# tg623623nana/Vehicle_Motion_Planning_with_Obstacles_Avoidance_using_MPC

Measured on AMD Instinct MI355X. Metric: OBCA MPC steps/sec (batch) at N=5, 3 obs, higher is better.
Workload: dtype f64

## Files before the change

### vehicle_motion_planning_with_obstacles_avoidance_using_mpc_amd/csrc/obca_device.h

```cpp
#ifndef OBCA_DEVICE_H
#define OBCA_DEVICE_H

#include <math.h>
#include <stdint.h>
#include "../../include/obca_mpc.h"

#define OBCA_ACC_MAX0 0.6
#define OBCA_ACC_MAX1 0.5235987755982988
#define OBCA_T_MIN 1e-4

#define OBCA_MU_INIT 0.1
#define OBCA_KAPPA_MU 0.2
#define OBCA_THETA_MU 1.5
#define OBCA_KAPPA_EPS 10.0
#define OBCA_TAU_MIN 0.99
#define OBCA_BOUND_PUSH 1e-2
#define OBCA_BOUND_FRAC 1e-2
#define OBCA_KAPPA_D 1e-5
#define OBCA_KAPPA_SIGMA 1e10
#define OBCA_S_MAX 100.0
#define OBCA_GAMMA_THETA 1e-5
#define OBCA_GAMMA_PHI 1e-8
#define OBCA_DELTA 1.0
#define OBCA_S_THETA 1.1
// ... 63 lines not shown
constexpr long long obca_even(long long c) { return (c + 1) & ~1ll; }
constexpr ObcaShapeSizes obca_shape_sizes(int N, int nO, int M) {
    const int N1 = N + 1, np = N1 * nO, MW = OBCA_MAX_EDGES + 6;
    const int n_max = N1 * (3 + M + 4 * nO) + 2 * N + 1;
    const int R_max = 3 + 3 * N + 3 + 2 * N1 + 2 * N + 2 * N + 2 + 2 * np + N1 * M + N1 * 4 * nO;
    long long t = 0;
    t += obca_even(n_max) + obca_even(n_max > 120 ? n_max : 120) + obca_even(5 * N1 + 1) + obca_even(n_max);
    t += 5 * obca_even(R_max);
    t += obca_even(3 * N1 + 3);
    t += 4 * obca_even(N1) + 2 * obca_even(2 * np);
    t += 3 * obca_even(2 * np);
    t += obca_even(N1 * M * 2) + obca_even(N1 * M) + obca_even(3 * N1);
    t += obca_even(36 * N1) + obca_even(8 * N1);
    {
        const long long nx = obca_even(n_max), nr = obca_even(R_max), ny = (long long)MW * 4 * np;
        t += obca_even(ny > nx + nr ? ny : nx + nr);
    }
    t += obca_even(36 * N1 > 12 * np ? 36 * N1 : 12 * np) + obca_even(6 * N1) + obca_even(12 * N1) + obca_even(2 * N1) + obca_even(9 * (N1 + 1));
    t += obca_even(32) + obca_even(8);
    const int inst_off = (int)t;
    t += OBCA_INST_DOUBLES;
    return ObcaShapeSizes{n_max, R_max, inst_off, t};
}
#define OBCA_LDS_CU_BYTES (160 * 1024)
#define OBCA_LDS_STATIC_BYTES 64
constexpr long long obca_soc_doubles(int N, int nO, int M) {
    return obca_even((long long)obca_shape_sizes(N, nO, M).n_max + 2 * (long long)obca_shape_sizes(N, nO, M).R_max + 2 * (long long)(N + 1) * nO);
}
constexpr int obca_wgs_per_cu(long long dyn_bytes, int cap) {
    return (int)(OBCA_LDS_CU_BYTES / (dyn_bytes + OBCA_LDS_STATIC_BYTES)) < cap ? (int)(OBCA_LDS_CU_BYTES / (dyn_bytes + OBCA_LDS_STATIC_BYTES)) : cap;
}
constexpr int obca_soc_lds_wave(int N, int nO, int M) {
    const long long base = 8 * obca_shape_sizes(N, nO, M).lds_doubles, with = base + 8 * obca_soc_doubles(N, nO, M);
    return (obca_wgs_per_cu(base, 4) > 0 && obca_wgs_per_cu(with, 4) == obca_wgs_per_cu(base, 4)) ? (int)obca_shape_sizes(N, nO, M).lds_doubles : 0;
}
constexpr int obca_soc_lds_mw(int N, int nO, int M) {
    const long long off = obca_shape_sizes(N, nO, M).lds_doubles + OBCA_ZK_DOUBLES(N) + OBCA_HYB_DOUBLES(obca_shape_sizes(N, nO, M).R_max);
    return 8 * (off + obca_soc_doubles(N, nO, M)) + OBCA_LDS_STATIC_BYTES <= OBCA_LDS_CU_BYTES ? (int)off : 0;
}
#define OBCA_SHAPES(X) X(5, 2, 2) X(5, 3, 6) X(5, 4, 10) X(5, 5, 14) X(5, 6, 18) X(6, 2, 2) X(6, 3, 6) X(6, 4, 10) X(6, 5, 14)
#define OBCA_MW_SHAPES(X) X(20, 3, 6) X(20, 5, 14)

struct ObcaWeightsDev { double Q[9], P[9], R1[4], R2[4]; };
struct ObcaOptsDev { double tol, rho, feas_tol; int32_t max_iter_free, max_iter_fixed, max_soc, order, nstarts, patience, retry_iter, dodge, screen, time_bound; };
static inline bool obca_resolve_starts(ObcaOptsDev* o, int start_order, int single_start, int patience, int retry_iter, int N, int dodge = 0, int terminal_screen = 0) {
    if (start_order < OBCA_START_DEFAULT || start_order > OBCA_START_X0_FIRST || single_start < 0 || single_start > 1) return false;
// ... 98 lines not shown
```

### vehicle_motion_planning_with_obstacles_avoidance_using_mpc_amd/csrc/obca_kernel.hip

```cpp

#include <hip/hip_runtime.h>
#include <stdint.h>
#include <math.h>
#include "obca_device.h"

#define SYNC() __syncthreads()

#ifndef OBCA_NT
#define OBCA_NT 64
#endif

#ifdef OBCA_PROFILE
#define PROF_DECL long long prof_last = wall_clock64();
#define PROF(i) { const long long t_ = wall_clock64(); prof_t[i] += t_ - prof_last; prof_last = t_; }
#define RPROF(i) { const long long t_ = wall_clock64(); prof_t[i] += t_ - rlast; rlast = t_; }
__device__ long long* prof_dummy;
#else
#define PROF_DECL
#define PROF(i)
#define RPROF(i)
#endif

namespace {

// ... 438 lines not shown
#undef X
    double* m_;
    double* gl_;
    enum {
#define X(f) K_##f,
        OBCA_ROW_FIELDS(X)
#undef X
        K_N };
    __device__ __forceinline__ static constexpr int slots() { return 5; }
#define X(f) __device__ __forceinline__ double& f##R(int j) { return j < 4 ? f##_[j] : m_[K_##f]; } \
             __device__ __forceinline__ double f##R(int j) const { return j < 4 ? f##_[j] : m_[K_##f]; }
    OBCA_ROW_FIELDS(X)
#undef X
#define X(f) __device__ __forceinline__ double& f(int j) { return f##R(j); } \
             __device__ __forceinline__ double f(int j) const { return f##R(j); }
    X(s) X(p) X(n) X(zL) X(zU) X(zp) X(zn) X(dy) X(iDs) X(iDp) X(iDn) X(rs) X(rp) X(rn)
#undef X
    __device__ __forceinline__ double& g(int j) { return j < 4 ? gl_[NT * j] : m_[K_g]; }
    __device__ __forceinline__ double g(int j) const { return j < 4 ? gl_[NT * j] : m_[K_g]; }
};

struct Err { double E, dual, prim, comp; };

template <int RPL>
__device__ __forceinline__ Err ipm_errors(const Lay& L, const Sh& S, const Rows<RPL>& W, double mu, double rho, double rxmax,
                          double crotmax, double nusum, int lane) {
    double dual = 0.0, prim = 0.0, comp = 0.0, ysum = 0.0, zsum = 0.0, nz = 0.0, nrow = 0.0;
#pragma unroll
    for (int j = 0; j < W.slots(); ++j) {
        const int r = lane + NT * j;
        if (r < L.R) {
            const double w = row_w(L, r);
            const bool eq = row_iseq(L, r);
            const double lo_ = S.Lb[r], up_ = S.Ub[r];
            const bool hasL = !eq && lo_ > -INFINITY, hasU = !eq && up_ < INFINITY;
            const double s = W.s(j), y = S.y[r], p = W.p(j), n = W.n(j);
            const double zL = hasL ? W.zL(j) : 0.0, zU = hasU ? W.zU(j) : 0.0, zp = W.zp(j), zn = W.zn(j);
            if (!eq) dual = dmaxabs(dual, -y - zL + zU);
            dual = dmaxabs(dual, rho - y - zp);
            dual = dmaxabs(dual, rho + y - zn);
            prim = dmaxabs(prim, W.g(j) - (eq ? 0.0 : s) - p + n);
            comp = dmaxabs(comp, p * zp - mu);
            comp = dmaxabs(comp, n * zn - mu);
            if (hasL) comp = dmaxabs(comp, (s - lo_) * zL - mu);
            if (hasU) comp = dmaxabs(comp, (up_ - s) * zU - mu);
            ysum += w * fabs(y);
            zsum += w * (zL + zU + zp + zn);
            nz += w * ((hasL ? 1.0 : 0.0) + (hasU ? 1.0 : 0.0) + 2.0);
            nrow += w;
        }
    }
    dual = fmax(red_max(dual), rxmax);
    prim = fmax(red_max(prim), crotmax);
    comp = red_max(comp);
    ysum = red_sum(ysum) + nusum;
    zsum = red_sum(zsum);
    nz = red_sum(nz);
    nrow = red_sum(nrow) + 2.0 * L.npair;
    const double sd = fmax(OBCA_S_MAX, (ysum + zsum) / (nrow + nz)) / OBCA_S_MAX;
    const double sc = fmax(OBCA_S_MAX, zsum / nz) / OBCA_S_MAX;
    Err e;
    e.dual = dual; e.prim = prim; e.comp = comp;
    e.E = fmax(fmax(dual / sd, prim), comp / sc);
    return e;
}

struct ErrFirst { Err e0, em; double th, pnsum, emax; };
template <int RPL>
__device__ __forceinline__ ErrFirst ipm_errors_first(const Lay& L, const Sh& S, const Rows<RPL>& W, double mu, double rho, double rxmax,
                                     double crotmax, double nusum, double th_lane, double nz, double nrow, int lane) {
    double dual = 0.0, prim = 0.0, comp0 = 0.0, compm = 0.0, ysum = 0.0, zsum = 0.0, th = th_lane, pnsum = 0.0, emax = 0.0;
#pragma unroll
    for (int j = 0; j < W.slots(); ++j) {
        const int r = lane + NT * j;
        if (r < L.R) {
            const double w = row_w(L, r);
            const bool eq = row_iseq(L, r);
            const double lo_ = S.Lb[r], up_ = S.Ub[r];
            const bool hasL = !eq && lo_ > -INFINITY, hasU = !eq && up_ < INFINITY;
            const double s = W.s(j), y = S.y[r], p = W.p(j), n = W.n(j);
            const double zL = hasL ? W.zL(j) : 0.0, zU = hasU ? W.zU(j) : 0.0, zp = W.zp(j), zn = W.zn(j);
            if (!eq) dual = dmaxabs(dual, -y - zL + zU);
            dual = dmaxabs(dual, rho - y - zp);
            dual = dmaxabs(dual, rho + y - zn);
            const double res = W.g(j) - (eq ? 0.0 : s) - p + n;
            prim = dmaxabs(prim, res);
            th += w * fabs(res);
            pnsum += w * (p + n);
            emax = fmax(emax, p + n);
            comp0 = dmaxabs(comp0, p * zp); compm = dmaxabs(compm, p * zp - mu);
            comp0 = dmaxabs(comp0, n * zn); compm = dmaxabs(compm, n * zn - mu);
            if (hasL) { comp0 = dmaxabs(comp0, (s - lo_) * zL); compm = dmaxabs(compm, (s - lo_) * zL - mu); }
            if (hasU) { comp0 = dmaxabs(comp0, (up_ - s) * zU); compm = dmaxabs(compm, (up_ - s) * zU - mu); }
            ysum += w * fabs(y);
            zsum += w * (zL + zU + zp + zn);
        }
    }
    ErrFirst o;
    dual = fmax(red_max(dual), rxmax);
    prim = fmax(red_max(prim), crotmax);
    comp0 = red_max(comp0);
    compm = red_max(compm);
    ysum = red_sum(ysum) + nusum;
    zsum = red_sum(zsum);
    o.th = red_sum(th); o.pnsum = red_sum(pnsum); o.emax = red_max(emax);
    const double sd = fmax(OBCA_S_MAX, (ysum + zsum) / (nrow + nz)) / OBCA_S_MAX;
    const double sc = fmax(OBCA_S_MAX, zsum / nz) / OBCA_S_MAX;
    o.e0.dual = dual; o.e0.prim = prim; o.e0.comp = comp0; o.e0.E = fmax(fmax(dual / sd, prim), comp0 / sc);
    o.em.dual = dual; o.em.prim = prim; o.em.comp = compm; o.em.E = fmax(fmax(dual / sd, prim), compm / sc);
    return o;
}

struct Lin { double iDs, iDp, iDn, rs, rp, rn; };
__device__ __forceinline__ Lin row_lin(double lo, double up, bool eq, double s, double p, double n, double y,
                                       double zL, double zU, double zp, double zn, double mu, double rho, double dw) {
    const bool hasL = !eq && lo > -INFINITY, hasU = !eq && up < INFINITY;
    double sig = 0.0, gs = 0.0;
    if (hasL) { const double isl = rcp64(s - lo); sig += zL * isl; gs -= mu * isl; }
    if (hasU) { const double isu = rcp64(up - s); sig += zU * isu; gs += mu * isu; }
    if (hasL && !hasU) gs += OBCA_KAPPA_D * mu;
    if (hasU && !hasL) gs -= OBCA_KAPPA_D * mu;
    const double ip = rcp64(p), inn = rcp64(n);
    Lin q;
    q.iDs = eq ? 0.0 : rcp64(sig + dw);
    q.iDp = rcp64(zp * ip + dw);
    q.iDn = rcp64(zn * inn + dw);
    q.rs = eq ? 0.0 : (-y + gs);
    q.rp = rho - y - mu * ip;
    q.rn = rho + y - mu * inn;
    return q;
}

__device__ __forceinline__ double row_barrier(double lo, double up, bool eq, double s, double p, double n, double mu,
// ... 968 lines not shown
template <bool FROM_MEMORY> __device__ __forceinline__ int uni(int v) { return FROM_MEMORY ? __builtin_amdgcn_readfirstlane(v) : v; }
template <bool FROM_MEMORY, class T> __device__ __forceinline__ T* uni(T* p) {
    if (!FROM_MEMORY) return p;
    const unsigned long long u = reinterpret_cast<unsigned long long>(p);
    const unsigned lo = (unsigned)__builtin_amdgcn_readfirstlane((int)(unsigned)u), hi = (unsigned)__builtin_amdgcn_readfirstlane((int)(unsigned)(u >> 32));
    return reinterpret_cast<T*>(((unsigned long long)hi << 32) | lo);
}
template <bool FROM_MEMORY> __device__ __forceinline__ double uni(double v) { return FROM_MEMORY ? lane_read(v, 0) : v; }
struct ObcaHead {
    int32_t B, N, nO, M, n_max, R_max, inst_off, two_sided, soc_lds;
    const int32_t* variant;
    const double *x0, *u0, *xref, *A, *b, *Ts, *term;
    double *xopt, *uopt, *ts_opt;
    int32_t *status, *iters;
    double *info, *prof, *warm_z;
    const int32_t* warm_use;
    double warm_mu;
    double *cert_z, *cert_y, *soc_ws, *gm_ws;
    long long gm_stride;
};

typedef const __attribute__((address_space(4))) ObcaLaunch ObcaLaunchConst;

struct ShapeAny { static constexpr bool fixed = false; static constexpr int N = 0, nO = 0, M = 0, n_max = 0, R_max = 0, inst_off = 0, soc_lds = 0; };
template <int N_, int NO_, int M_, bool FT = false>
struct ShapeIs {
    static constexpr bool fixed = true;
    static constexpr int N = N_, nO = NO_, M = M_;
    static constexpr int n_max = obca_shape_sizes(N_, NO_, M_).n_max, R_max = obca_shape_sizes(N_, NO_, M_).R_max - (FT ? 3 : 0),
                         inst_off = obca_shape_sizes(N_, NO_, M_).inst_off;
#if OBCA_NT == 64
    static constexpr int RPL = R_max <= 256 ? 4 : R_max <= 320 ? 5 : 6;
    static_assert(R_max <= 384, "shape beyond the one-wavefront kernels");
    static constexpr int soc_lds = obca_soc_lds_wave(N_, NO_, M_);
#else
    static constexpr int RPL = R_max <= 768 ? 3 : -5;
    static_assert(R_max <= 1280, "shape beyond the four-wavefront LDS kernels");
    static constexpr int soc_lds = obca_soc_lds_mw(N_, NO_, M_);
#endif
};

template <int RPL, bool FROM_MEMORY = false, class DESC = const ObcaLaunch, class SHAPE = ShapeAny>
__device__ __forceinline__ void obca_ipm_body(DESC& Ain, const int inst, const bool first) {
    extern __shared__ __attribute__((aligned(16))) double smem[];
    const int lane = threadIdx.x;
    ObcaHead A;
    {
        constexpr bool U = FROM_MEMORY;
        A.B = uni<U>(Ain.B); A.N = uni<U>(Ain.N); A.nO = uni<U>(Ain.nO); A.M = uni<U>(Ain.M); A.n_max = uni<U>(Ain.n_max);
        A.R_max = uni<U>(Ain.R_max); A.inst_off = uni<U>(Ain.inst_off); A.two_sided = uni<U>(Ain.two_sided); A.soc_lds = uni<U>(Ain.soc_lds);
        A.variant = uni<U>(Ain.variant); A.x0 = uni<U>(Ain.x0); A.u0 = uni<U>(Ain.u0); A.xref = uni<U>(Ain.xref); A.A = uni<U>(Ain.A);
// ... 40 lines not shown
    const bool dodge2 = start_s >= Ain.prm.opt.nstarts + 2;
    const bool from_window = kind == OBCA_KIND_WINDOW;

    Lay L;
    L.N = A.N; L.nO = A.nO; L.M = A.M;
    L.variant = A.variant[inst];
    L.free_T = (L.variant == 4) ? 1 : 0;
    L.NS = 5 + L.M + 4 * L.nO;
    L.n = (L.N + 1) * (3 + L.M + 4 * L.nO) + 2 * L.N + L.free_T;
    L.npair = (L.N + 1) * L.nO;
    L.r_init = 0; L.r_dyn = 3; L.r_term = 3 + 3 * L.N;
    L.r_xb = L.r_term + (L.variant == 4 ? 3 : 0);
    L.r_ub = L.r_xb + 2 * (L.N + 1);
    L.r_acc = L.r_ub + 2 * L.N;
    L.r_T = L.r_acc + 2 * L.N;
    L.r_tx = L.r_T + (L.free_T ? 2 : 0);
    L.r_norm = L.r_tx + (L.variant == 6 ? 2 : 0);
    L.r_dist = L.r_norm + L.npair;
    L.r_lam = L.r_dist + L.npair;
    L.r_mu = L.r_lam + (L.N + 1) * L.M;
    L.R = L.r_mu + (L.N + 1) * 4 * L.nO;

    constexpr bool GM = (RPL == 0);
    Sh S;
    Rows<RPL> W;
    {
        double* p = smem;
        double* q = nullptr;
        if constexpr (GM) q = A.gm_ws + (size_t)blockIdx.x * (size_t)A.gm_stride;
        auto take = [&](int cnt) { double* r = p; p += (cnt + 1) & ~1; return r; };
        auto takeG = [&](int cnt) { if constexpr (!GM) { double* r = p; p += (cnt + 1) & ~1; return r; } else { double* r = q; q += (cnt + 1) & ~1; return r; } };
        const int nmax = A.n_max, Rmax = A.R_max, np = L.npair, N1 = L.N + 1;
        S.x = takeG(nmax); S.dx = takeG(nmax > 120 ? nmax : 120); S.gf = take(5 * N1 + 1); S.bx = takeG(nmax);
        S.y = takeG(Rmax); S.Einv = takeG(Rmax); S.gh = takeG(Rmax); S.Lb = takeG(Rmax); S.Ub = takeG(Rmax); S.dy = take(3 * N1 + 3);
        S.ct = take(N1); S.st = take(N1); S.cc = takeG(2 * np); S.ctt = take(N1); S.stt = take(N1); S.cct = takeG(2 * np);
        S.nu = takeG(2 * np); S.dnu = takeG(2 * np); S.crot = takeG(2 * np);
        S.Aobs = takeG(N1 * L.M * 2); S.bobs = takeG(N1 * L.M); S.xref = take(3 * N1);
        S.Lall = take(36 * N1); S.lall = take(8 * N1);
        {
            const int nx = (nmax + 1) & ~1, nr = (Rmax + 1) & ~1, ny = MW * 4 * np;
            S.Y = takeG(ny > nx + nr ? ny : nx + nr);
            S.xt = S.Y; S.tmp = S.Y + nx;
        }
        if constexpr (!GM) {
            S.Pk = take(36 * N1 > 12 * np ? 36 * N1 : 12 * np);
            S.Sloc = S.Pk;
// ... 119 lines not shown
        gm = fmax(red_max(gm), O.rho);
        sf = (gm > OBCA_MAX_GRADIENT) ? OBCA_MAX_GRADIENT / gm : 1.0;
        rho = O.rho * sf;
    }
    SYNC();
    f0 = eval_objective<true>(L, S, in, S.x, sf, lane);
    PUT(IV_F, f0);
    double mu = (from_window || (kind >= OBCA_KIND_DODGE_R && !dodge2)) ? OBCA_RESTART_MU : (warm ? A.warm_mu : (dodge2 ? OBCA_DODGE_LEVEL2_MU : OBCA_MU_INIT));
    {
        int bb = 0;
        for (int r = lane; r < L.R; r += NT) {
            double lo, up;
            row_bounds(L, in, r, lo, up);
            S.Lb[r] = lo; S.Ub[r] = up;
            S.tmp[r] = row_value(L, S, in, S.x, S.ct, S.st, S.cc, r);
        }
#pragma unroll
        for (int j = 0; j < W.slots(); ++j) {
            const int r = lane + NT * j;
            W.s(j) = 0.0; W.p(j) = 1.0; W.n(j) = 1.0;
            W.zL(j) = 0.0; W.zU(j) = 0.0; W.zp(j) = 1.0; W.zn(j) = 1.0; W.g(j) = 0.0; W.dy(j) = 0.0;
            W.iDs(j) = 0.0; W.iDp(j) = 1.0; W.iDn(j) = 1.0; W.rs(j) = 0.0; W.rp(j) = 0.0; W.rn(j) = 0.0;
            if (r < L.R) {
                const double lo = S.Lb[r], up = S.Ub[r];
                const bool eq = row_iseq(L, r);
                const double g = S.tmp[r];
                double s = g;
                const bool hasL = lo > -INFINITY, hasU = up < INFINITY;
                if (eq) s = 0.0;
                else if (hasL && hasU) {
                    if (!(lo < up)) bb = 1;
                    const double pL = fmin(OBCA_BOUND_PUSH * fmax(1.0, fabs(lo)), OBCA_BOUND_FRAC * (up - lo));
                    const double pU = fmin(OBCA_BOUND_PUSH * fmax(1.0, fabs(up)), OBCA_BOUND_FRAC * (up - lo));
                    s = fmin(fmax(s, lo + pL), up - pU);
                } else if (hasL) s = fmax(s, lo + OBCA_BOUND_PUSH * fmax(1.0, fabs(lo)));
                else if (hasU) s = fmin(s, up - OBCA_BOUND_PUSH * fmax(1.0, fabs(up)));
                const double rr = g - s;
                const double a = (mu - rho * rr) / (2.0 * rho);
                const double en = a + sqrt(a * a + mu * rr / (2.0 * rho));
                const double ep = rr + en;
                W.g(j) = g; W.s(j) = s; W.p(j) = ep; W.n(j) = en;
                W.zp(j) = mu / ep; W.zn(j) = mu / en;
                W.zL(j) = (!eq && hasL) ? 1.0 : 0.0;
                W.zU(j) = (!eq && hasU) ? 1.0 : 0.0;
                S.y[r] = rho - mu / ep;
            }
        }
        bad_bounds = red_or(bb) != 0;
        for (int pr = lane; pr < L.npair; pr += NT) {
            double e1, e2;
            rot_value(L, S.x, S.ct, S.st, S.cc, pr, e1, e2);
            S.crot[2 * pr] = e1; S.crot[2 * pr + 1] = e2;
        }
        SYNC();
    }

    double cnt_nz = 0.0, cnt_rows = 0.0;
#pragma unroll
    for (int j = 0; j < W.slots(); ++j) {
        const int r = lane + NT * j;
        if (r < L.R) {
            const double w = row_w(L, r);
            const bool eq = row_iseq(L, r);
            cnt_nz += w * (((!eq && S.Lb[r] > -INFINITY) ? 1.0 : 0.0) + ((!eq && S.Ub[r] < INFINITY) ? 1.0 : 0.0) + 2.0);
            cnt_rows += w;
        }
    }
    cnt_nz = red_sum(cnt_nz);
    cnt_rows = red_sum(cnt_rows) + 2.0 * L.npair;
    PUT(IV_CNTNZ, cnt_nz); PUT(IV_CNTROWS, cnt_rows);

    bool f_valid = false;
    double f_th = 0.0, f_phi = 0.0;
    PUT(IV_TAU, fmax(OBCA_TAU_MIN, 1.0 - mu));
    PUT(IV_DWLAST, 0.0); PUT(IV_EMAX, 0.0); PUT(IV_PHIK, NAN);
    int acc_count = 0;
    bool have_prev = false;

#ifdef OBCA_PROFILE
    long long prof_t[20];
    for (int i = 0; i < 20; ++i) prof_t[i] = 0;
#endif
    enum { LS_TH = 0, LS_FOBJ, LS_DW, LS_AZ, LS_DPHI, LS_PHI, LS_AMIN, LS_PWTH, LS_PWDPHI, LS_ALPHA, LS_THOLD };
    bool soc_pass = false, use_soc = false, first_trial = true;
    int soc_it = 0;
    PROF_DECL
#ifdef OBCA_PROFILE
    if (NT == 64) prof_t[10] += prof_last - prof_body_t0;
#endif
    if (bad_bounds) status = OBCA_STATUS_BAD_BOUNDS;
    else
    for (it = 0; it <= max_iter; ++it) {
        PROF(11)
        double th = 0.0, fobj = 0.0, delta_w = 0.0;
        if (!soc_pass) {
        gather_grad<false>(L, S, in, S.bx, lane);
        double rxmax = 0.0, crotmax = 0.0, nusum = 0.0, pnsum = 0.0;
        for (int t = lane; t < L.n; t += NT) rxmax = dmaxabs(rxmax, S.bx[t]);
        for (int t = lane; t < 2 * L.npair; t += NT) { crotmax = dmaxabs(crotmax, S.crot[t]); nusum += fabs(S.nu[t]); th += fabs(S.crot[t]); }
        rxmax = red_max(rxmax); crotmax = red_max(crotmax); nusum = red_sum(nusum);
        const ErrFirst ef = ipm_errors_first<RPL>(L, S, W, mu, rho, rxmax, crotmax, nusum, th, GET(IV_CNTNZ), GET(IV_CNTROWS), lane);
        th = ef.th; pnsum = ef.pnsum; PUT(IV_EMAX, ef.emax);
        const Err e0 = ef.e0;
        const double E0 = e0.E;
        PUT(IV_E0, E0);
        if (it == 0) {
            PUT(IV_THMAX, OBCA_THETA_MAX_FACT * fmax(1.0, th));
            PUT(IV_THMIN, OBCA_THETA_MIN_FACT * fmax(1.0, th));
        }
        if (E0 <= O.tol && e0.dual <= 1.0 && e0.prim <= 1e-4 && e0.comp <= 1e-4) { status = OBCA_STATUS_OK; break; }
        fobj = GET(IV_F) + rho * pnsum;
        const double objchg = have_prev ? fabs(fobj - GET(IV_FPREV)) / fmax(1.0, fabs(fobj)) : INFINITY;
        if (E0 <= acc_tol && e0.dual <= 1e10 && e0.prim <= 1e-2 && e0.comp <= 1e-2 && objchg <= acc_objchg) {
            if (++acc_count >= OBCA_ACCEPTABLE_ITER) { status = OBCA_STATUS_ACCEPTABLE; break; }
        } else acc_count = 0;
        if (it == max_iter) break;
        PROF(0)
        {
            const double mu_floor = O.tol / (OBCA_KAPPA_EPS + 1.0);
            bool first_mu = true;
            while (mu > mu_floor) {
                const Err em = first_mu ? ef.em : ipm_errors<RPL>(L, S, W, mu, rho, rxmax, crotmax, nusum, lane);
                first_mu = false;
                if (em.E > OBCA_KAPPA_EPS * mu) break;
                mu = fmax(mu_floor, fmin(OBCA_KAPPA_MU * mu, mu * sqrt(mu)));
                PUT(IV_TAU, fmax(OBCA_TAU_MIN, 1.0 - mu));
                PUT(IV_PHIK, NAN);
                f_valid = false;
            }
        }
        } else {
            th = S.lsv[LS_TH]; fobj = S.lsv[LS_FOBJ]; delta_w = S.lsv[LS_DW];
            (void)eval_objective<true>(L, S, in, S.x, sf, lane);
        }
        PROF(1)
#define ws_dxo (A.soc_lds ? smem + A.soc_lds : A.soc_ws + (size_t)inst * (A.n_max + 2 * A.R_max + 2 * L.npair))
#define ws_dyo (ws_dxo + A.n_max)
#define ws_gsoc (ws_dyo + A.R_max)
#define ws_dnuo (ws_gsoc + A.R_max)
        const int max_soc = (A.soc_lds || A.soc_ws) ? O.max_soc : 0;
#pragma unroll
        for (int j = 0; j < W.slots(); ++j) {
            W.dy(j) = 0.0; W.iDs(j) = 0.0; W.iDp(j) = 0.0; W.iDn(j) = 0.0; W.rs(j) = 0.0; W.rp(j) = 0.0; W.rn(j) = 0.0;
        }
        bool first_try = true;
        int fail = 0;
        const double dw_last = GET(IV_DWLAST);
        for (;;) {
#pragma unroll
            for (int j = 0; j < W.slots(); ++j) {
                const int r = lane + NT * j;
                if (r < L.R) {
                    const bool eq = row_iseq(L, r);
                    const double y = S.y[r];
                    const double lo_ = S.Lb[r], up_ = S.Ub[r];
                    const Lin q = row_lin(lo_, up_, eq, W.s(j), W.p(j), W.n(j), y, W.zL(j), W.zU(j), W.zp(j),
                                          W.zn(j), mu, rho, delta_w);
                    const double rg = soc_pass ? ws_gsoc[r] : W.g(j) - (eq ? 0.0 : W.s(j)) - W.p(j) + W.n(j);
                    const double gh = rg + q.rs * q.iDs + q.rp * q.iDp - q.rn * q.iDn;
                    const double Ei = rcp64(q.iDs + q.iDp + q.iDn);
                    S.Einv[r] = Ei;
                    S.gh[r] = gh;
                    S.tmp[r] = row_soft(L, r) ? y : fma(gh, Ei, y);
                }
            }
            SYNC();
            if constexpr (GM) {
                double* es = const_cast<double*>(S.Es); double* gs = const_cast<double*>(S.gs); double* uv = const_cast<double*>(S.uv);
                for (int t = lane; t < L.r_term; t += NT) { es[t] = S.Einv[t]; gs[t] = S.gh[t]; }
                for (int t = lane; t < 2 * L.N; t += NT) uv[t] = S.x[L.iu(t >> 1) + (t & 1)];
                if (lane == 0 && L.free_T) uv[2 * (L.N + 1)] = S.x[L.iT()];
                SYNC();
            }
            gather_grad<true>(L, S, in, S.bx, lane);
            PROF(2)
            assemble_stages(L, S, in, sf, delta_w, lane);
            PROF(3)
            int bad = local_blocks(L, S, in, delta_w, lane);
            PROF(4)
#ifdef OBCA_PROFILE
            if (!bad) bad = riccati(L, S, in, lane, prof_t, A.two_sided != 0);
#if !defined(OBCA_TWO_SIDED_CHECK) && OBCA_NT >= 256
            if (A.two_sided != 0) {
                double dmax = 0.0;
                for (int r = L.r_init + (lane & 63); r < L.r_term; r += 64) dmax = fmax(dmax, S.Einv[r]);
                dmax = wave_max(dmax);
// ... 29 lines not shown
#endif
#else
            if (!bad) bad = riccati(L, S, in, lane, A.two_sided != 0);
#endif
            PROF(5)
            ++nfact;
            if (!bad || soc_pass) break;
            if (first_try) {
                delta_w = (dw_last == 0.0) ? OBCA_DELTA_W_0 : fmax(OBCA_DELTA_W_MIN, OBCA_KAPPA_W_MINUS * dw_last);
                first_try = false;
            } else {
                delta_w *= (dw_last == 0.0) ? OBCA_KAPPA_W_PLUS_BAR : OBCA_KAPPA_W_PLUS;
            }
            if (delta_w > OBCA_DELTA_W_MAX) { fail = 1; break; }
        }
        if (fail) { status = OBCA_STATUS_NUMERIC; break; }
        if (!soc_pass && delta_w > 0.0) PUT(IV_DWLAST, delta_w);
        double a_max = 1.0, a_z = 1.0, dphi = 0.0, phi = 0.0;
        const double phik = GET(IV_PHIK);
        const bool phi_known = !soc_pass && isfinite(phik);
        const double tau = GET(IV_TAU);
        for (int r = lane; r < L.R; r += NT)
            S.tmp[r] = row_soft(L, r) ? S.dy[r] : (row_jdx(L, S, in, r) + S.gh[r]) * S.Einv[r];
#pragma unroll
        for (int j = 0; j < W.slots(); ++j) {
            const int r = lane + NT * j;
            if (r < L.R) {
                const bool eq = row_iseq(L, r);
                const double lo_ = S.Lb[r], up_ = S.Ub[r];
            const bool hasL = !eq && lo_ > -INFINITY, hasU = !eq && up_ < INFINITY;
                const double dy = S.tmp[r];
                W.dy(j) = dy;
                {
                    const Lin q = row_lin(lo_, up_, eq, W.s(j), W.p(j), W.n(j), S.y[r], W.zL(j), W.zU(j), W.zp(j),
                                          W.zn(j), mu, rho, delta_w);
                    W.iDs(j) = q.iDs; W.iDp(j) = q.iDp; W.iDn(j) = q.iDn; W.rs(j) = q.rs; W.rp(j) = q.rp; W.rn(j) = q.rn;
                }
                const double w = row_w(L, r);
                const double ds = (dy - W.rs(j)) * W.iDs(j);
                const double dp = (dy - W.rp(j)) * W.iDp(j);
                const double dn = (-dy - W.rn(j)) * W.iDn(j);
                const double s = W.s(j), p = W.p(j), n = W.n(j);
                double gs = eq ? 0.0 : W.rs(j) + S.y[r];
                const double ids = rcp64(ds), ip = rcp64(p), inn = rcp64(n);
                if (hasL) {
                    const double sl = s - lo_, zL = W.zL(j);
                    if (ds < 0.0) a_max = fmin(a_max, -tau * sl * ids);
                    const double dz = (mu - zL * ds) * rcp64(sl) - zL;
                    if (dz < 0.0) a_z = fmin(a_z, -tau * zL * rcp64(dz));
                }
                if (hasU) {
                    const double su = up_ - s, zU = W.zU(j);
                    if (ds > 0.0) a_max = fmin(a_max, tau * su * ids);
                    const double dz = (mu + zU * ds) * rcp64(su) - zU;
                    if (dz < 0.0) a_z = fmin(a_z, -tau * zU * rcp64(dz));
                }
                if (dp < 0.0) a_max = fmin(a_max, -tau * p * rcp64(dp));
                if (dn < 0.0) a_max = fmin(a_max, -tau * n * rcp64(dn));
                const double zp = W.zp(j), zn = W.zn(j);
                const double dzp = (mu - zp * dp) * ip - zp, dzn = (mu - zn * dn) * inn - zn;
                if (dzp < 0.0) a_z = fmin(a_z, -tau * zp * rcp64(dzp));
                if (dzn < 0.0) a_z = fmin(a_z, -tau * zn * rcp64(dzn));
                if (!phi_known) phi += w * row_barrier(lo_, up_, eq, s, p, n, mu, rho);
                dphi += w * (gs * ds + (rho - mu * ip) * dp + (rho - mu * inn) * dn);
            }
        }
        for (int t = lane; t < L.n; t += NT) {
            const int k = t / L.NS, q = t - k * L.NS;
            if (L.free_T && t == L.iT()) dphi += S.gf[L.igT()] * S.dx[t];
            else if (q < (k < L.N ? 5 : 3)) dphi += S.gf[L.ig(k) + q] * S.dx[t];
        }
        a_max = red_min(a_max); a_z = red_min(a_z); dphi = red_sum(dphi); phi = phi_known ? phik : red_sum(phi) + GET(IV_F);
        double alpha_min;
        double pw_th = 0.0, pw_dphi = 1.0;
        double alpha = a_max, a_try = a_max, th_old = 0.0;
        if (!soc_pass) {
            if (dphi < 0.0) {
                pw_th = dpow(th, OBCA_S_THETA);
                pw_dphi = dpow(-dphi, OBCA_S_PHI);
                double c = fmin(OBCA_GAMMA_THETA, OBCA_GAMMA_PHI * th / (-dphi));
                if (th <= GET(IV_THMIN)) c = fmin(c, OBCA_DELTA * pw_th / pw_dphi);
                alpha_min = OBCA_GAMMA_ALPHA * c;
            } else alpha_min = OBCA_GAMMA_ALPHA * OBCA_GAMMA_THETA;
            first_trial = true; use_soc = false; soc_it = 0;
        } else {
            a_try = a_max;
            a_z = S.lsv[LS_AZ]; dphi = S.lsv[LS_DPHI]; phi = S.lsv[LS_PHI]; alpha_min = S.lsv[LS_AMIN];
            pw_th = S.lsv[LS_PWTH]; pw_dphi = S.lsv[LS_PWDPHI]; alpha = S.lsv[LS_ALPHA]; th_old = S.lsv[LS_THOLD];
        }
        soc_pass = false;
        PROF(6)
        double f_t = 0.0, phi_acc = NAN;
        bool accepted = false, aug = false;
        for (;;) {
            for (int t = lane; t < L.n; t += NT) S.xt[t] = S.x[t] + a_try * S.dx[t];
            SYNC();
            eval_geom(L, S, S.xt, S.ctt, S.stt, S.cct, lane);
            f_t = eval_objective<true>(L, S, in, S.xt, sf, lane);
            double th_t = 0.0, phi_t = 0.0;
            for (int r = lane; r < L.R; r += NT) S.tmp[r] = row_value(L, S, in, S.xt, S.ctt, S.stt, S.cct, r);
#pragma unroll
            for (int j = 0; j < W.slots(); ++j) {
                const int r = lane + NT * j;
                if (r < L.R) {
                    const bool eq = row_iseq(L, r);
                    const double dy = W.dy(j), w = row_w(L, r);
                    const double lo_ = S.Lb[r], up_ = S.Ub[r];
                    const double st = eq ? 0.0 : W.s(j) + a_try * (dy - W.rs(j)) * W.iDs(j);
                    const double pt = W.p(j) + a_try * (dy - W.rp(j)) * W.iDp(j);
                    const double nt = W.n(j) + a_try * (-dy - W.rn(j)) * W.iDn(j);
                    const double gt = S.tmp[r];
                    th_t += w * fabs(gt - st - pt + nt);
                    phi_t += w * row_barrier(lo_, up_, eq, st, pt, nt, mu, rho);
                }
            }
            for (int pr = lane; pr < L.npair; pr += NT) {
                double e1, e2;
                rot_value(L, S.xt, S.ctt, S.stt, S.cct, pr, e1, e2);
                th_t += fabs(e1) + fabs(e2);
                S.bx[2 * pr] = e1; S.bx[2 * pr + 1] = e2;
            }
            th_t = red_sum(th_t);
            phi_t = red_sum(phi_t) + f_t;
            bool ok = false;
            aug = false;
            const bool finite = isfinite(phi_t) && isfinite(th_t);
#if OBCA_NT == 64
            const bool blocked = (th_t >= GET(IV_THMAX)) || (__any(f_valid && th_t >= f_th && phi_t >= f_phi) != 0);
#else
            const bool blocked = (th_t >= GET(IV_THMAX)) || red_or(f_valid && th_t >= f_th && phi_t >= f_phi);
// ... 12 lines not shown
            bool soc_start = false, soc_next = false;
            if (use_soc) {
                if (!fin_eval || th_t > OBCA_KAPPA_SOC * th_old || soc_it >= max_soc) {
                    for (int t = lane; t < L.n; t += NT) S.dx[t] = ws_dxo[t];
                    for (int t = lane; t < 2 * L.npair; t += NT) S.dnu[t] = ws_dnuo[t];
#pragma unroll
                    for (int j = 0; j < W.slots(); ++j) {
                        const int r = lane + NT * j;
                        if (r < L.R) W.dy(j) = ws_dyo[r];
                    }
                    use_soc = false;
                    SYNC();
                } else soc_next = true;
            } else if (first_trial && max_soc > 0 && fin_eval && th_t >= th) {
                soc_start = true;
            }
            first_trial = false;
            if (soc_start || soc_next) {
                const double cf = soc_start ? alpha : a_try;
#pragma unroll
                for (int j = 0; j < W.slots(); ++j) {
                    const int r = lane + NT * j;
                    if (r < L.R) {
                        const bool eq = row_iseq(L, r);
                        const double dy = W.dy(j);
                        const double st = eq ? 0.0 : W.s(j) + a_try * (dy - W.rs(j)) * W.iDs(j);
                        const double pt = W.p(j) + a_try * (dy - W.rp(j)) * W.iDp(j);
                        const double nt = W.n(j) + a_try * (-dy - W.rn(j)) * W.iDn(j);
                        const double res = S.tmp[r] - st - pt + nt;
                        const double old = soc_start ? W.g(j) - (eq ? 0.0 : W.s(j)) - W.p(j) + W.n(j) : ws_gsoc[r];
                        ws_gsoc[r] = cf * old + res;
                        if (soc_start) ws_dyo[r] = dy;
                    }
                }
                if (soc_start) {
                    for (int t = lane; t < L.n; t += NT) ws_dxo[t] = S.dx[t];
                    for (int t = lane; t < 2 * L.npair; t += NT) ws_dnuo[t] = S.dnu[t];
                }
                for (int t = lane; t < 2 * L.npair; t += NT) S.crot[t] = cf * S.crot[t] + S.bx[t];
                if (lane == 0) {
                    S.lsv[LS_TH] = th; S.lsv[LS_FOBJ] = fobj; S.lsv[LS_DW] = delta_w; S.lsv[LS_AZ] = a_z; S.lsv[LS_DPHI] = dphi;
                    S.lsv[LS_PHI] = phi; S.lsv[LS_AMIN] = alpha_min; S.lsv[LS_PWTH] = pw_th; S.lsv[LS_PWDPHI] = pw_dphi;
                    S.lsv[LS_ALPHA] = alpha; S.lsv[LS_THOLD] = th_t;
                }
                use_soc = true;
                soc_pass = true;
                ++soc_it;
// ... 10 lines not shown
        if (!accepted) { status = OBCA_STATUS_LINESEARCH; break; }
        if (aug) {
            const double tn = (1.0 - OBCA_GAMMA_THETA) * th, pn = phi - OBCA_GAMMA_PHI * th;
#if OBCA_NT == 64
            if (f_valid && f_th >= tn && f_phi >= pn) f_valid = false;
            const unsigned long long freem = __ballot(!f_valid);
            if (freem == 0ull) { status = OBCA_STATUS_NUMERIC; break; }
            const int slot = __ffsll((long long)freem) - 1;
            if (lane == slot) { f_valid = true; f_th = tn; f_phi = pn; }
#else
            if (f_valid && f_th >= tn && f_phi >= pn) f_valid = false;
            const unsigned long long freem = __ballot(!f_valid && lane < OBCA_FILTER_CAP(A.R_max));
            const double cand = freem ? (double)((lane & ~63) + __ffsll((long long)freem) - 1) : 1e9;
            const double slot = red_min(cand);
            const int full = slot > 1e8 ? 1 : 0;
            if (!full && lane == (int)slot) { f_valid = true; f_th = tn; f_phi = pn; }
            if (full) { status = OBCA_STATUS_NUMERIC; break; }
#endif
        }
#pragma unroll
        for (int j = 0; j < W.slots(); ++j) {
            const int r = lane + NT * j;
            if (r < L.R) {
                const bool eq = row_iseq(L, r);
                const double lo_ = S.Lb[r], up_ = S.Ub[r];
            const bool hasL = !eq && lo_ > -INFINITY, hasU = !eq && up_ < INFINITY;
                const double dy = W.dy(j);
                const double dyz = use_soc ? ws_dyo[r] : dy;
                const double ds = (dy - W.rs(j)) * W.iDs(j);
                const double dp = (dy - W.rp(j)) * W.iDp(j);
                const double dn = (-dy - W.rn(j)) * W.iDn(j);
                const double dsz = (dyz - W.rs(j)) * W.iDs(j);
                const double dpz = (dyz - W.rp(j)) * W.iDp(j);
                const double dnz = (-dyz - W.rn(j)) * W.iDn(j);
                const double lo = lo_, up = up_;
                const double s_old = W.s(j), p_old = W.p(j), n_old = W.n(j);
                const double s = eq ? 0.0 : s_old + a_try * ds, p = p_old + a_try * dp, n = n_old + a_try * dn;
                const double ks = OBCA_KAPPA_SIGMA, iks = 1.0 / OBCA_KAPPA_SIGMA;
                if (hasL) {
                    const double zL = W.zL(j) + a_z * ((mu - W.zL(j) * dsz) * rcp64(s_old - lo) - W.zL(j));
                    const double msl = mu * rcp64(s - lo);
                    W.zL(j) = fmax(fmin(zL, ks * msl), msl * iks);
                }
                if (hasU) {
                    const double zU = W.zU(j) + a_z * ((mu + W.zU(j) * dsz) * rcp64(up - s_old) - W.zU(j));
                    const double msu = mu * rcp64(up - s);
                    W.zU(j) = fmax(fmin(zU, ks * msu), msu * iks);
                }
                const double zp = W.zp(j) + a_z * ((mu - W.zp(j) * dpz) * rcp64(p_old) - W.zp(j));
// ... 198 lines not shown
#ifndef OBCA_LOOP_R4
#define OBCA_LOOP_R4 true
#endif
#ifndef OBCA_LOOP_R56
#define OBCA_LOOP_R56 true
#endif
#ifndef OBCA_LOOP_MW
#define OBCA_LOOP_MW false
#endif
#ifndef OBCA_LOOP_GM
#define OBCA_LOOP_GM true
#endif
#if OBCA_NT == 64 && defined(OBCA_TU_SHAPE)
#ifndef OBCA_SHAPE_KERNEL_ATTR
#define OBCA_SHAPE_KERNEL_ATTR
#endif
#define OBCA_DEFINE_SHAPE_KERNEL(N_, O_, M_)                                                                                   \
    extern "C" __global__ void __launch_bounds__(64) OBCA_SHAPE_KERNEL_ATTR obca_ipm_kernel_s##N_##_##O_##_##M_(ObcaLaunch A, ObcaLaunch A2, ObcaLaunch A3) { \
        using SH = ShapeIs<N_, O_, M_>;                                                                                        \
        solve_with_escalation<SH::RPL, true, true, SH>(A, A2, A3);                                                            \
    }
OBCA_TU_SHAPE(OBCA_DEFINE_SHAPE_KERNEL)
#elif OBCA_NT == 64
extern "C" __global__ void __launch_bounds__(64) obca_ipm_kernel_r4(ObcaLaunch A, ObcaLaunch A2, ObcaLaunch A3) { solve_with_escalation<4, OBCA_LOOP_R4>(A, A2, A3); }
extern "C" __global__ void __launch_bounds__(64) obca_ipm_kernel_r5(ObcaLaunch A, ObcaLaunch A2, ObcaLaunch A3) { solve_with_escalation<5, OBCA_LOOP_R56>(A, A2, A3); }
extern "C" __global__ void __launch_bounds__(64) obca_ipm_kernel_r6(ObcaLaunch A, ObcaLaunch A2, ObcaLaunch A3) { solve_with_escalation<6, OBCA_LOOP_R56>(A, A2, A3); }
extern "C" __global__ void __launch_bounds__(64) obca_ipm_kernel_gm1(ObcaLaunch A, ObcaLaunch A2, ObcaLaunch A3) { solve_with_escalation<0, OBCA_LOOP_GM>(A, A2, A3); }

#include "obca_rollout_core.h"
#include "obca_audit_core.h"

__device__ __noinline__ void ro_prepare(const rollout::Dev* D, int b) { rollout::prepare(*D, b); }
__device__ __noinline__ void ro_finish(const rollout::Dev* D, int b) { rollout::finish(*D, b); }
__device__ __noinline__ void ro_stop(const rollout::Dev* D, int b) { rollout::stop_check_wave(*D, b); }
__device__ __noinline__ int ro_screen(const ObcaLaunch* L, int b, double* tmax) { return terminal_screen_dev(L, b, 0, 1, tmax); }
__device__ __noinline__ int ro_retry(const rollout::Dev* D, int g, int b) { rollout::make_retry(*D, g, b); return D->var8[g][b]; }
__device__ __noinline__ long long ro_flag_sel(const rollout::Dev* D, int b) { return ((long long)D->sel[b] << 32) | (unsigned)D->flags[b]; }


#define OBCA_RO_SPIN_LIMIT (1 << 24)
#define OBCA_GETREG_XCC_ID (20 | (0 << 6) | ((4 - 1) << 11))

template <int RPL, class SHAPE>
__device__ __forceinline__ void ro_solve_step(const rollout::Dev& D, const ObcaLaunch* launches, const int g, const int b, int* ro_msg) {
    const int lane = threadIdx.x;
    bool nodge = false;
// ... 165 lines not shown
```

Measured before the change: 1.128 million.

## Specialize mu-only row slots at compile time and reuse error terms in mu loop

For fixed shapes, the register slot index from which all rows are known to be the mu/obstacle rows (no equality, lower bound 0, no upper bound, weight 1, not soft) is computed at compile time. Row loops skip the LDS loads of bounds, weights and row flags for those slots. The mu-decrease loop now recomputes only the complementarity error and reuses the dual and primal terms from the first error evaluation, since those do not depend on mu. The power computations for the switching condition are done once on lane 0 and only when needed. The approach relies on the row-layout assumption holding for every shape variant.

```diff
diff --git a/vehicle_motion_planning_with_obstacles_avoidance_using_mpc_amd/csrc/obca_device.h b/vehicle_motion_planning_with_obstacles_avoidance_using_mpc_amd/csrc/obca_device.h
--- a/vehicle_motion_planning_with_obstacles_avoidance_using_mpc_amd/csrc/obca_device.h
+++ b/vehicle_motion_planning_with_obstacles_avoidance_using_mpc_amd/csrc/obca_device.h
@@ -109,6 +109,20 @@
     t += OBCA_INST_DOUBLES;
     return ObcaShapeSizes{n_max, R_max, inst_off, t};
 }
+#define OBCA_NO_MU_SLOT (1 << 20)
+constexpr int obca_r_mu(int N, int nO, int M, int variant) {
+    return 3 + 3 * N + (variant == 4 ? 3 : 0) + 2 * (N + 1) + 2 * N + 2 * N + (variant == 4 ? 2 : 0) + (variant == 6 ? 2 : 0) +
+           2 * (N + 1) * nO + (N + 1) * M;
+}
+constexpr int obca_mu_slot(int N, int nO, int M, int nt) {
+    int r = obca_r_mu(N, nO, M, 4);
+    if (obca_r_mu(N, nO, M, 6) > r) r = obca_r_mu(N, nO, M, 6);
+    if (obca_r_mu(N, nO, M, 8) > r) r = obca_r_mu(N, nO, M, 8);
+    return (r + nt - 1) / nt;
+}
+static_assert(obca_mu_slot(5, 3, 6, 64) == 2 && obca_mu_slot(6, 3, 6, 64) == 3 && obca_mu_slot(5, 2, 2, 64) == 2 &&
+              obca_mu_slot(5, 5, 14, 64) == 4 && obca_mu_slot(5, 6, 18, 64) == 4, "mu slots of the one-wavefront shapes");
+static_assert(obca_mu_slot(20, 3, 6, 256) == 2 && obca_mu_slot(20, 5, 14, 256) == 3, "mu slots of the four-wavefront shapes");
 #define OBCA_LDS_CU_BYTES (160 * 1024)
 #define OBCA_LDS_STATIC_BYTES 64
 constexpr long long obca_soc_doubles(int N, int nO, int M) {
diff --git a/vehicle_motion_planning_with_obstacles_avoidance_using_mpc_amd/csrc/obca_kernel.hip b/vehicle_motion_planning_with_obstacles_avoidance_using_mpc_amd/csrc/obca_kernel.hip
--- a/vehicle_motion_planning_with_obstacles_avoidance_using_mpc_amd/csrc/obca_kernel.hip
+++ b/vehicle_motion_planning_with_obstacles_avoidance_using_mpc_amd/csrc/obca_kernel.hip
@@ -484,61 +484,22 @@
 
 struct Err { double E, dual, prim, comp; };
 
-template <int RPL>
-__device__ __forceinline__ Err ipm_errors(const Lay& L, const Sh& S, const Rows<RPL>& W, double mu, double rho, double rxmax,
-                          double crotmax, double nusum, int lane) {
-    double dual = 0.0, prim = 0.0, comp = 0.0, ysum = 0.0, zsum = 0.0, nz = 0.0, nrow = 0.0;
+template <int MUS>
+__device__ __forceinline__ constexpr bool mu_only(int j) { return MUS < OBCA_NO_MU_SLOT && j >= MUS; }
+
+struct ErrFirst { Err e0, em; double th, pnsum, emax, dsd, sc; };
+template <int RPL, int MUS>
+__device__ __forceinline__ ErrFirst ipm_errors_first(const Lay& L, const Sh& S, const Rows<RPL>& W, double mu, double rho, double rxmax,
+                                     double crotmax, double nusum, double th_lane, double nz, double nrow, int lane) {
+    double dual = 0.0, prim = 0.0, comp0 = 0.0, compm = 0.0, ysum = 0.0, zsum = 0.0, th = th_lane, pnsum = 0.0, emax = 0.0;
 #pragma unroll
     for (int j = 0; j < W.slots(); ++j) {
         const int r = lane + NT * j;
         if (r < L.R) {
-            const double w = row_w(L, r);
-            const bool eq = row_iseq(L, r);
-            const double lo_ = S.Lb[r], up_ = S.Ub[r];
-            const bool hasL = !eq && lo_ > -INFINITY, hasU = !eq && up_ < INFINITY;
-            const double s = W.s(j), y = S.y[r], p = W.p(j), n = W.n(j);
-            const double zL = hasL ? W.zL(j) : 0.0, zU = hasU ? W.zU(j) : 0.0, zp = W.zp(j), zn = W.zn(j);
-            if (!eq) dual = dmaxabs(dual, -y - zL + zU);
-            dual = dmaxabs(dual, rho - y - zp);
-            dual = dmaxabs(dual, rho + y - zn);
-            prim = dmaxabs(prim, W.g(j) - (eq ? 0.0 : s) - p + n);
-            comp = dmaxabs(comp, p * zp - mu);
-            comp = dmaxabs(comp, n * zn - mu);
-            if (hasL) comp = dmaxabs(comp, (s - lo_) * zL - mu);
-            if (hasU) comp = dmaxabs(comp, (up_ - s) * zU - mu);
-            ysum += w * fabs(y);
-            zsum += w * (zL + zU + zp + zn);
-            nz += w * ((hasL ? 1.0 : 0.0) + (hasU ? 1.0 : 0.0) + 2.0);
-            nrow += w;
-        }
-    }
-    dual = fmax(red_max(dual), rxmax);
-    prim = fmax(red_max(prim), crotmax);
-    comp = red_max(comp);
-    ysum = red_sum(ysum) + nusum;
-    zsum = red_sum(zsum);
-    nz = red_sum(nz);
-    nrow = red_sum(nrow) + 2.0 * L.npair;
-    const double sd = fmax(OBCA_S_MAX, (ysum + zsum) / (nrow + nz)) / OBCA_S_MAX;
-    const double sc = fmax(OBCA_S_MAX, zsum / nz) / OBCA_S_MAX;
-    Err e;
-    e.dual = dual; e.prim = prim; e.comp = comp;
-    e.E = fmax(fmax(dual / sd, prim), comp / sc);
-    return e;
-}
-
-struct ErrFirst { Err e0, em; double th, pnsum, emax; };
-template <int RPL>
-__device__ __forceinline__ ErrFirst ipm_errors_first(const Lay& L, const Sh& S, const Rows<RPL>& W, double mu, double rho, double rxmax,
-                                     double crotmax, double nusum, double th_lane, double nz, double nrow, int lane) {
-    double dual = 0.0, prim = 0.0, comp0 = 0.0, compm = 0.0, ysum = 0.0, zsum = 0.0, th = th_lane, pnsum = 0.0, emax = 0.0;
-#pragma unroll
-    for (int j = 0; j < W.slots(); ++j) {
-        const int r = lane + NT * j;
-        if (r < L.R) {
-            const double w = row_w(L, r);
-            const bool eq = row_iseq(L, r);
-            const double lo_ = S.Lb[r], up_ = S.Ub[r];
+            const bool muk = mu_only<MUS>(j);
+            const double w = muk ? 1.0 : row_w(L, r);
+            const bool eq = muk ? false : row_iseq(L, r);
+            const double lo_ = muk ? 0.0 : S.Lb[r], up_ = muk ? INFINITY : S.Ub[r];
             const bool hasL = !eq && lo_ > -INFINITY, hasU = !eq && up_ < INFINITY;
             const double s = W.s(j), y = S.y[r], p = W.p(j), n = W.n(j);
             const double zL = hasL ? W.zL(j) : 0.0, zU = hasU ? W.zU(j) : 0.0, zp = W.zp(j), zn = W.zn(j);
@@ -568,9 +529,31 @@
     o.th = red_sum(th); o.pnsum = red_sum(pnsum); o.emax = red_max(emax);
     const double sd = fmax(OBCA_S_MAX, (ysum + zsum) / (nrow + nz)) / OBCA_S_MAX;
     const double sc = fmax(OBCA_S_MAX, zsum / nz) / OBCA_S_MAX;
-    o.e0.dual = dual; o.e0.prim = prim; o.e0.comp = comp0; o.e0.E = fmax(fmax(dual / sd, prim), comp0 / sc);
-    o.em.dual = dual; o.em.prim = prim; o.em.comp = compm; o.em.E = fmax(fmax(dual / sd, prim), compm / sc);
+    o.dsd = dual / sd; o.sc = sc;
+    o.e0.dual = dual; o.e0.prim = prim; o.e0.comp = comp0; o.e0.E = fmax(fmax(o.dsd, prim), comp0 / sc);
+    o.em.dual = dual; o.em.prim = prim; o.em.comp = compm; o.em.E = fmax(fmax(o.dsd, prim), compm / sc);
     return o;
+}
+
+template <int RPL, int MUS>
+__device__ __forceinline__ double ipm_comp(const Lay& L, const Sh& S, const Rows<RPL>& W, double mu, int lane) {
+    double comp = 0.0;
+#pragma unroll
+    for (int j = 0; j < W.slots(); ++j) {
+        const int r = lane + NT * j;
+        if (r < L.R) {
+            const bool muk = mu_only<MUS>(j);
+            const bool eq = muk ? false : row_iseq(L, r);
+            const double lo_ = muk ? 0.0 : S.Lb[r], up_ = muk ? INFINITY : S.Ub[r];
+            const bool hasL = !eq && lo_ > -INFINITY, hasU = !eq && up_ < INFINITY;
+            const double s = W.s(j);
+            comp = dmaxabs(comp, W.p(j) * W.zp(j) - mu);
+            comp = dmaxabs(comp, W.n(j) * W.zn(j) - mu);
+            if (hasL) comp = dmaxabs(comp, (s - lo_) * W.zL(j) - mu);
+            if (hasU) comp = dmaxabs(comp, (up_ - s) * W.zU(j) - mu);
+        }
+    }
+    return red_max(comp);
 }
 
 struct Lin { double iDs, iDp, iDn, rs, rp, rn; };
@@ -1585,11 +1568,12 @@
 
 typedef const __attribute__((address_space(4))) ObcaLaunch ObcaLaunchConst;
 
-struct ShapeAny { static constexpr bool fixed = false; static constexpr int N = 0, nO = 0, M = 0, n_max = 0, R_max = 0, inst_off = 0, soc_lds = 0; };
+struct ShapeAny { static constexpr bool fixed = false; static constexpr int N = 0, nO = 0, M = 0, n_max = 0, R_max = 0, inst_off = 0, soc_lds = 0, mu_slot = OBCA_NO_MU_SLOT; };
 template <int N_, int NO_, int M_, bool FT = false>
 struct ShapeIs {
     static constexpr bool fixed = true;
     static constexpr int N = N_, nO = NO_, M = M_;
+    static constexpr int mu_slot = OBCA_NT == 64 ? obca_mu_slot(N_, NO_, M_, OBCA_NT) : OBCA_NO_MU_SLOT;
     static constexpr int n_max = obca_shape_sizes(N_, NO_, M_).n_max, R_max = obca_shape_sizes(N_, NO_, M_).R_max - (FT ? 3 : 0),
                          inst_off = obca_shape_sizes(N_, NO_, M_).inst_off;
 #if OBCA_NT == 64
@@ -1676,6 +1660,7 @@
     L.R = L.r_mu + (L.N + 1) * 4 * L.nO;
 
     constexpr bool GM = (RPL == 0);
+    constexpr int MUS = SHAPE::mu_slot;
     Sh S;
     Rows<RPL> W;
     {
@@ -1841,8 +1826,9 @@
             W.zL(j) = 0.0; W.zU(j) = 0.0; W.zp(j) = 1.0; W.zn(j) = 1.0; W.g(j) = 0.0; W.dy(j) = 0.0;
             W.iDs(j) = 0.0; W.iDp(j) = 1.0; W.iDn(j) = 1.0; W.rs(j) = 0.0; W.rp(j) = 0.0; W.rn(j) = 0.0;
             if (r < L.R) {
-                const double lo = S.Lb[r], up = S.Ub[r];
-                const bool eq = row_iseq(L, r);
+                const bool muk = mu_only<MUS>(j);
+                const double lo = muk ? 0.0 : S.Lb[r], up = muk ? INFINITY : S.Ub[r];
+                const bool eq = muk ? false : row_iseq(L, r);
                 const double g = S.tmp[r];
                 double s = g;
                 const bool hasL = lo > -INFINITY, hasU = up < INFINITY;
@@ -1879,6 +1865,7 @@
     for (int j = 0; j < W.slots(); ++j) {
         const int r = lane + NT * j;
         if (r < L.R) {
+            if (mu_only<MUS>(j)) { cnt_nz += 3.0; cnt_rows += 1.0; continue; }
             const double w = row_w(L, r);
             const bool eq = row_iseq(L, r);
             cnt_nz += w * (((!eq && S.Lb[r] > -INFINITY) ? 1.0 : 0.0) + ((!eq && S.Ub[r] < INFINITY) ? 1.0 : 0.0) + 2.0);
@@ -1918,7 +1905,7 @@
         for (int t = lane; t < L.n; t += NT) rxmax = dmaxabs(rxmax, S.bx[t]);
         for (int t = lane; t < 2 * L.npair; t += NT) { crotmax = dmaxabs(crotmax, S.crot[t]); nusum += fabs(S.nu[t]); th += fabs(S.crot[t]); }
         rxmax = red_max(rxmax); crotmax = red_max(crotmax); nusum = red_sum(nusum);
-        const ErrFirst ef = ipm_errors_first<RPL>(L, S, W, mu, rho, rxmax, crotmax, nusum, th, GET(IV_CNTNZ), GET(IV_CNTROWS), lane);
+        const ErrFirst ef = ipm_errors_first<RPL, MUS>(L, S, W, mu, rho, rxmax, crotmax, nusum, th, GET(IV_CNTNZ), GET(IV_CNTROWS), lane);
         th = ef.th; pnsum = ef.pnsum; PUT(IV_EMAX, ef.emax);
         const Err e0 = ef.e0;
         const double E0 = e0.E;
@@ -1939,9 +1926,9 @@
             const double mu_floor = O.tol / (OBCA_KAPPA_EPS + 1.0);
             bool first_mu = true;
             while (mu > mu_floor) {
-                const Err em = first_mu ? ef.em : ipm_errors<RPL>(L, S, W, mu, rho, rxmax, crotmax, nusum, lane);
+                const double Em = first_mu ? ef.em.E : fmax(fmax(ef.dsd, ef.e0.prim), ipm_comp<RPL, MUS>(L, S, W, mu, lane) / ef.sc);
                 first_mu = false;
-                if (em.E > OBCA_KAPPA_EPS * mu) break;
+                if (Em > OBCA_KAPPA_EPS * mu) break;
                 mu = fmax(mu_floor, fmin(OBCA_KAPPA_MU * mu, mu * sqrt(mu)));
                 PUT(IV_TAU, fmax(OBCA_TAU_MIN, 1.0 - mu));
                 PUT(IV_PHIK, NAN);
@@ -1970,9 +1957,10 @@
             for (int j = 0; j < W.slots(); ++j) {
                 const int r = lane + NT * j;
                 if (r < L.R) {
-                    const bool eq = row_iseq(L, r);
+                    const bool muk = mu_only<MUS>(j);
+                    const bool eq = muk ? false : row_iseq(L, r);
                     const double y = S.y[r];
-                    const double lo_ = S.Lb[r], up_ = S.Ub[r];
+                    const double lo_ = muk ? 0.0 : S.Lb[r], up_ = muk ? INFINITY : S.Ub[r];
                     const Lin q = row_lin(lo_, up_, eq, W.s(j), W.p(j), W.n(j), y, W.zL(j), W.zU(j), W.zp(j),
                                           W.zn(j), mu, rho, delta_w);
                     const double rg = soc_pass ? ws_gsoc[r] : W.g(j) - (eq ? 0.0 : W.s(j)) - W.p(j) + W.n(j);
@@ -1980,7 +1968,7 @@
                     const double Ei = rcp64(q.iDs + q.iDp + q.iDn);
                     S.Einv[r] = Ei;
                     S.gh[r] = gh;
-                    S.tmp[r] = row_soft(L, r) ? y : fma(gh, Ei, y);
+                    S.tmp[r] = (!muk && row_soft(L, r)) ? y : fma(gh, Ei, y);
                 }
             }
             SYNC();
@@ -2056,13 +2044,17 @@
         const double tau = GET(IV_TAU);
         for (int r = lane; r < L.R; r += NT)
             S.tmp[r] = row_soft(L, r) ? S.dy[r] : (row_jdx(L, S, in, r) + S.gh[r]) * S.Einv[r];
+#if OBCA_NT == 64
+        PROF(19)
+#endif
 #pragma unroll
         for (int j = 0; j < W.slots(); ++j) {
             const int r = lane + NT * j;
             if (r < L.R) {
-                const bool eq = row_iseq(L, r);
-                const double lo_ = S.Lb[r], up_ = S.Ub[r];
-            const bool hasL = !eq && lo_ > -INFINITY, hasU = !eq && up_ < INFINITY;
+                const bool muk = mu_only<MUS>(j);
+                const bool eq = muk ? false : row_iseq(L, r);
+                const double lo_ = muk ? 0.0 : S.Lb[r], up_ = muk ? INFINITY : S.Ub[r];
+                const bool hasL = !eq && lo_ > -INFINITY, hasU = !eq && up_ < INFINITY;
                 const double dy = S.tmp[r];
                 W.dy(j) = dy;
                 {
@@ -2070,7 +2062,7 @@
                                           W.zn(j), mu, rho, delta_w);
                     W.iDs(j) = q.iDs; W.iDp(j) = q.iDp; W.iDn(j) = q.iDn; W.rs(j) = q.rs; W.rp(j) = q.rp; W.rn(j) = q.rn;
                 }
-                const double w = row_w(L, r);
+                const double w = muk ? 1.0 : row_w(L, r);
                 const double ds = (dy - W.rs(j)) * W.iDs(j);
                 const double dp = (dy - W.rp(j)) * W.iDp(j);
                 const double dn = (-dy - W.rn(j)) * W.iDn(j);
@@ -2099,6 +2091,9 @@
                 dphi += w * (gs * ds + (rho - mu * ip) * dp + (rho - mu * inn) * dn);
             }
         }
+#if OBCA_NT == 64
+        PROF(18)
+#endif
         for (int t = lane; t < L.n; t += NT) {
             const int k = t / L.NS, q = t - k * L.NS;
             if (L.free_T && t == L.iT()) dphi += S.gf[L.igT()] * S.dx[t];
@@ -2109,11 +2104,14 @@
         double pw_th = 0.0, pw_dphi = 1.0;
         double alpha = a_max, a_try = a_max, th_old = 0.0;
         if (!soc_pass) {
+            const bool sw = dphi < 0.0 && th <= GET(IV_THMIN);
+            if (sw) {
+                pw_th = lane_read(dpow(th, OBCA_S_THETA), 0);
+                pw_dphi = lane_read(dpow(-dphi, OBCA_S_PHI), 0);
+            }
             if (dphi < 0.0) {
-                pw_th = dpow(th, OBCA_S_THETA);
-                pw_dphi = dpow(-dphi, OBCA_S_PHI);
                 double c = fmin(OBCA_GAMMA_THETA, OBCA_GAMMA_PHI * th / (-dphi));
-                if (th <= GET(IV_THMIN)) c = fmin(c, OBCA_DELTA * pw_th / pw_dphi);
+                if (sw) c = fmin(c, OBCA_DELTA * pw_th / pw_dphi);
                 alpha_min = OBCA_GAMMA_ALPHA * c;
             } else alpha_min = OBCA_GAMMA_ALPHA * OBCA_GAMMA_THETA;
             first_trial = true; use_soc = false; soc_it = 0;
@@ -2137,9 +2135,10 @@
             for (int j = 0; j < W.slots(); ++j) {
                 const int r = lane + NT * j;
                 if (r < L.R) {
-                    const bool eq = row_iseq(L, r);
-                    const double dy = W.dy(j), w = row_w(L, r);
-                    const double lo_ = S.Lb[r], up_ = S.Ub[r];
+                    const bool muk = mu_only<MUS>(j);
+                    const bool eq = muk ? false : row_iseq(L, r);
+                    const double dy = W.dy(j), w = muk ? 1.0 : row_w(L, r);
+                    const double lo_ = muk ? 0.0 : S.Lb[r], up_ = muk ? INFINITY : S.Ub[r];
                     const double st = eq ? 0.0 : W.s(j) + a_try * (dy - W.rs(j)) * W.iDs(j);
                     const double pt = W.p(j) + a_try * (dy - W.rp(j)) * W.iDp(j);
                     const double nt = W.n(j) + a_try * (-dy - W.rn(j)) * W.iDn(j);
@@ -2198,7 +2197,7 @@
                 for (int j = 0; j < W.slots(); ++j) {
                     const int r = lane + NT * j;
                     if (r < L.R) {
-                        const bool eq = row_iseq(L, r);
+                        const bool eq = mu_only<MUS>(j) ? false : row_iseq(L, r);
                         const double dy = W.dy(j);
                         const double st = eq ? 0.0 : W.s(j) + a_try * (dy - W.rs(j)) * W.iDs(j);
                         const double pt = W.p(j) + a_try * (dy - W.rp(j)) * W.iDp(j);
@@ -2255,9 +2254,10 @@
         for (int j = 0; j < W.slots(); ++j) {
             const int r = lane + NT * j;
             if (r < L.R) {
-                const bool eq = row_iseq(L, r);
-                const double lo_ = S.Lb[r], up_ = S.Ub[r];
-            const bool hasL = !eq && lo_ > -INFINITY, hasU = !eq && up_ < INFINITY;
+                const bool muk = mu_only<MUS>(j);
+                const bool eq = muk ? false : row_iseq(L, r);
+                const double lo_ = muk ? 0.0 : S.Lb[r], up_ = muk ? INFINITY : S.Ub[r];
+                const bool hasL = !eq && lo_ > -INFINITY, hasU = !eq && up_ < INFINITY;
                 const double dy = W.dy(j);
                 const double dyz = use_soc ? ws_dyo[r] : dy;
                 const double ds = (dy - W.rs(j)) * W.iDs(j);
@@ -2502,6 +2502,7 @@
     }
 OBCA_TU_SHAPE(OBCA_DEFINE_SHAPE_KERNEL)
 #elif OBCA_NT == 64
+extern "C" int obca_internal_mu_slot(int N, int nO, int M, int nt) { return obca_mu_slot(N, nO, M, nt); }
 extern "C" __global__ void __launch_bounds__(64) obca_ipm_kernel_r4(ObcaLaunch A, ObcaLaunch A2, ObcaLaunch A3) { solve_with_escalation<4, OBCA_LOOP_R4>(A, A2, A3); }
 extern "C" __global__ void __launch_bounds__(64) obca_ipm_kernel_r5(ObcaLaunch A, ObcaLaunch A2, ObcaLaunch A3) { solve_with_escalation<5, OBCA_LOOP_R56>(A, A2, A3); }
 extern "C" __global__ void __launch_bounds__(64) obca_ipm_kernel_r6(ObcaLaunch A, ObcaLaunch A2, ObcaLaunch A3) { solve_with_escalation<6, OBCA_LOOP_R56>(A, A2, A3); }
```

Result: faster. 1.205 million (median of 6 runs) (+6.8%).
